# CoderLSF/fast-llama

Measured on AMD Instinct MI355X. Metric: decode tokens/s LLaMA2-7B int8, higher is better.
Workload: dtype int8; 1 GPU; LLaMA2-7B int8 .flm-layout synthetic weights (portable splitmix64 checkpoint, norm weights 1.0), single-stream greedy decode, prompt 9 tokens, positions 14..928, fp32 KV cache, max_seq 1024; parallelism=single-gpu

## Files before the change

fast-llama_amd/capi.py:

```python
from __future__ import annotations

import ctypes as C
import os

import numpy as np

_HERE = os.path.dirname(os.path.abspath(__file__))
LIB_PATH = os.environ.get("FLM_GPU_LIB") or os.path.join(_HERE, "lib", "libflm_gpu.so")

QT_NONE, QT_INT16, QT_INT8 = 0, 1, 2
KCLASSES = ("embed", "qkv", "attn", "attn_o", "ffn13", "ffn2", "cls", "argmax", "allreduce", "attn_wo", "ffn", "qkv_attn_wo", "layer", "back", "layers", "token")

SYMBOLS = (
    "flm_comm_unique_id", "flm_ctx_create", "flm_ctx_destroy", "flm_p2p_export", "flm_p2p_import", "flm_last_error", "flm_upload_tensor",
    "flm_forward", "flm_forward_argmax", "flm_decode_greedy", "flm_decode_timed", "flm_decode_timed_each", "flm_last_tokens", "flm_reset_kv", "flm_prepare", "flm_sync",
    "flm_kernel_times", "flm_kernel_bytes", "flm_set_option", "flm_query", "flm_debug_read",
    "flm_op_quantize", "flm_op_matmul_q", "flm_op_rmsnorm", "flm_op_swiglu", "flm_op_rope", "flm_op_softmax",
    "flm_op_attention", "flm_op_expf", "flm_op_math", "flm_op_square_sum", "flm_op_argmax", "flm_op_handoff_litmus", "flm_plan_shards",
)


TUNING_KEYS = ("wg_per_cu", "use_mfma", "tok_preq", "tok_nstq", "back_nst13", "back_nst13_head", "back_nst2", "back_pre13", "back_pre2", "back_ao2", "inject_wait_failure")


class FlmError(RuntimeError):
    pass


class ModelDesc(C.Structure):
    _fields_ = [(n, C.c_int32) for n in ("dim", "hidden_dim", "n_layers", "n_heads", "n_kv_heads", "vocab_size",
                                          "max_seq_len", "quant_type", "quant_group_size")]


class ShardPlan(C.Structure):
    _fields_ = [(n, C.c_int32) for n in ("head_begin", "head_count", "hidden_begin", "hidden_count", "dim_begin", "dim_count", "vocab_begin", "vocab_count")]


_lib = None


def lib():
    global _lib
    if _lib is None:
        if not os.path.exists(LIB_PATH):
            raise FlmError(f"{LIB_PATH} is missing: run `python -c 'import __graft_entry__ as g; g.build()'` (no CPU fallback exists)")
        _lib = C.CDLL(LIB_PATH, mode=C.RTLD_GLOBAL)
        _lib.flm_last_error.restype = C.c_char_p
        _lib.flm_last_error.argtypes = [C.c_void_p]
    return _lib


def _p(a):
    return a.ctypes.data_as(C.c_void_p) if a is not None else None


def _check(rc, ctx=None):
    if rc != 0:
        msg = lib().flm_last_error(ctx)
        raise FlmError(f"flm error {rc}: {msg.decode() if msg else ''}")


def desc_from_config(cfg, max_seq_len=1024) -> ModelDesc:
    return ModelDesc(cfg.dim, cfg.hidden_dim, cfg.n_layers, cfg.n_heads, cfg.n_kv_heads, cfg.vocab_size,
                     max_seq_len, cfg.quant_type, cfg.quant_group_size)


def plan_shards(desc: ModelDesc, rank: int, world: int) -> ShardPlan:
    out = ShardPlan()
    _check(lib().flm_plan_shards(C.byref(desc), rank, world, C.byref(out)))
    return out


def comm_unique_id() -> bytes:
    buf = C.create_string_buffer(128)
    _check(lib().flm_comm_unique_id(buf))
    return buf.raw


class Ctx:

    def __init__(self, desc: ModelDesc, device=0, rank=0, world=1, comm_id: bytes | None = None):
        self.desc = desc
        self._h = C.c_void_p()
        _check(lib().flm_ctx_create(C.byref(desc), device, rank, world, comm_id, C.byref(self._h)))

    def close(self):
        if self._h:
            lib().flm_ctx_destroy(self._h)
            self._h = C.c_void_p()

    def __del__(self):
        try:
            self.close()
        except Exception:
            pass

    def p2p_export(self) -> bytes:
        buf = C.create_string_buffer(128)
        _check(lib().flm_p2p_export(self._h, buf), self._h)
        return buf.raw

    def p2p_import(self, blobs):
        raw = b"".join(blobs)
        _check(lib().flm_p2p_import(self._h, raw, len(blobs)), self._h)

    @staticmethod
    def regroup(ctxs):
        blobs = [c.p2p_export() for c in ctxs]
        for c in ctxs:
            c.p2p_import(blobs)

    def upload(self, kind, layer, value):
        if isinstance(value, tuple):
            q, s = value
            q = np.ascontiguousarray(q); s = np.ascontiguousarray(s, dtype=np.float32)
            qt = QT_INT8 if q.dtype == np.int8 else QT_INT16
            _check(lib().flm_upload_tensor(self._h, kind, layer, qt, _p(q), _p(s), q.shape[0], q.shape[1]), self._h)
        else:
            v = np.ascontiguousarray(value, dtype=np.float32)
            rows, cols = v.shape if v.ndim == 2 else (1, v.shape[0])
            _check(lib().flm_upload_tensor(self._h, kind, layer, QT_NONE, _p(v), None, rows, cols), self._h)

    def upload_all(self, tensors):
        for (kind, layer), v in tensors.items():
            self.upload(kind, layer, v)

    def forward(self, tokens, pos) -> np.ndarray:
        t = np.ascontiguousarray(tokens, dtype=np.int32)
        out = np.empty(self.desc.vocab_size, dtype=np.float32)
        _check(lib().flm_forward(self._h, _p(t), len(t), int(pos), _p(out)), self._h)
        return out

    def forward_argmax(self, tokens, pos) -> int:
        t = np.ascontiguousarray(tokens, dtype=np.int32)
        nxt = C.c_int32(-1)
        _check(lib().flm_forward_argmax(self._h, _p(t), len(t), int(pos), C.byref(nxt)), self._h)
        return nxt.value

    def decode_greedy(self, first_token, pos, n_steps) -> np.ndarray:
        out = np.empty(n_steps, dtype=np.int32)
        _check(lib().flm_decode_greedy(self._h, int(first_token), int(pos), int(n_steps), _p(out)), self._h)
        return out

    def decode_timed(self, first_token, pos, n_steps) -> float:
        ms = C.c_float(0)
        _check(lib().flm_decode_timed(self._h, int(first_token), int(pos), int(n_steps), C.byref(ms)), self._h)
        return ms.value

    def decode_timed_each(self, first_token, pos, n_steps) -> np.ndarray:
        ms = np.zeros(n_steps, dtype=np.float32)
        _check(lib().flm_decode_timed_each(self._h, int(first_token), int(pos), int(n_steps), _p(ms)), self._h)
        return ms

    def last_tokens(self, n) -> np.ndarray:
        out = np.empty(n, dtype=np.int32)
        _check(lib().flm_last_tokens(self._h, int(n), _p(out)), self._h)
        return out

    def reset_kv(self):
        _check(lib().flm_reset_kv(self._h), self._h)

    def prepare(self):
        _check(lib().flm_prepare(self._h), self._h)

    def sync(self):
        _check(lib().flm_sync(self._h), self._h)

    def set_option(self, key, value, unlock=True):
        if unlock and key in TUNING_KEYS and not self.query("tuning"):
            _check(lib().flm_set_option(self._h, b"tuning", 1), self._h)
        _check(lib().flm_set_option(self._h, key.encode(), int(value)), self._h)

    def query(self, key) -> int:
        v = C.c_int(0)
        _check(lib().flm_query(self._h, key.encode(), C.byref(v)), self._h)
        return int(v.value)

    def debug_read(self, what, layer, n):
        names = {"x1": 0, "q": 1, "att_out": 2, "hd": 3, "kcache": 4, "vcache": 5, "logits": 6, "trace": 7, "trace_abs": 8, "back_trace": 10}
        out = np.empty(n, dtype=np.float32)
        _check(lib().flm_debug_read(self._h, names[what], int(layer), _p(out), C.c_size_t(n)), self._h)
        return out

    def kernel_times(self, pos, iters=3):
        avg = np.zeros(len(KCLASSES), dtype=np.float32); cnt = np.zeros(len(KCLASSES), dtype=np.int32)
        _check(lib().flm_kernel_times(self._h, int(pos), int(iters), _p(avg), _p(cnt)), self._h)
        return {k: (float(avg[i]), int(cnt[i])) for i, k in enumerate(KCLASSES)}

    def kernel_bytes(self, kclass, pos) -> float:
        b = C.c_double(0)
        _check(lib().flm_kernel_bytes(self._h, KCLASSES.index(kclass), int(pos), C.byref(b)), self._h)
        return b.value


def op_quantize(x, qt, gs=64):
    x = np.ascontiguousarray(x, dtype=np.float32)
    q = np.empty(x.size, dtype=np.int8 if qt == QT_INT8 else np.int16)
    s = np.empty(x.size // gs, dtype=np.float32)
    _check(lib().flm_op_quantize(qt, _p(q), _p(s), _p(x), C.c_size_t(x.size), gs))
    return q, s


def op_matmul_q(qt, W, sW, X, sX, gs=64):
    W = np.ascontiguousarray(W); X = np.ascontiguousarray(X)
    sW = np.ascontiguousarray(sW, dtype=np.float32); sX = np.ascontiguousarray(sX, dtype=np.float32)
    m, n = W.shape; w = X.shape[0]
    out = np.empty((w, m), dtype=np.float32)
    _check(lib().flm_op_matmul_q(qt, _p(out), _p(W), _p(sW), _p(X), _p(sX), m, n, w, gs))
    return out


def op_argmax(logits) -> int:
    a = np.ascontiguousarray(logits, dtype=np.float32)
    idx = C.c_int32(-1)
    _check(lib().flm_op_argmax(_p(a), int(a.size), C.byref(idx)))
    return idx.value


def op_handoff_litmus(rounds):
    bad, to = C.c_int(0), C.c_int(0)
    _check(lib().flm_op_handoff_litmus(int(rounds), C.byref(bad), C.byref(to)))
    return bad.value, to.value


def op_rmsnorm(x, w):
    x = np.ascontiguousarray(x, dtype=np.float32); w = np.ascontiguousarray(w, dtype=np.float32)
    o = np.empty_like(x)
    _check(lib().flm_op_rmsnorm(_p(o), _p(x), _p(w), C.c_size_t(x.size)))
    return o


def op_square_sum(x):
    x = np.ascontiguousarray(x, dtype=np.float32)
    o = np.empty(6, dtype=np.float32)
    _check(lib().flm_op_square_sum(_p(x), C.c_size_t(x.size), _p(o)))
    return o[0], o[1], o[2:6]


def op_swiglu(xo, xr):
    a = np.array(xo, dtype=np.float32, copy=True); b = np.ascontiguousarray(xr, dtype=np.float32)
    _check(lib().flm_op_swiglu(_p(a), _p(b), C.c_size_t(a.size)))
    return a


def op_rope(x, pos):
    x = np.ascontiguousarray(x, dtype=np.float32); o = np.empty_like(x)
    _check(lib().flm_op_rope(_p(o), _p(x), x.size, int(pos)))
    return o


def op_softmax(x, n=None):
    a = np.array(x, dtype=np.float32, copy=True)
    _check(lib().flm_op_softmax(_p(a), int(a.size if n is None else n)))
    return a


def op_expf(x):
    a = np.array(x, dtype=np.float32, copy=True).reshape(-1)
    _check(lib().flm_op_expf(_p(a), C.c_size_t(a.size)))
    return a


def op_math(fn, x, y=None):
    a = np.array(x, dtype=np.float32, copy=True).reshape(-1)
    b = None if y is None else np.ascontiguousarray(y, dtype=np.float32).reshape(-1)
    _check(lib().flm_op_math(int(fn), _p(a), _p(b), C.c_size_t(a.size)))
    return a


def op_attention(kc, vc, q, k, v, n_heads, hs, max_seq, pos):
    out = np.empty(n_heads * hs, dtype=np.float32)
    for a in (kc, vc):
        assert a.dtype == np.float32 and a.flags.c_contiguous
    q = np.ascontiguousarray(q, dtype=np.float32); k = np.ascontiguousarray(k, dtype=np.float32); v = np.ascontiguousarray(v, dtype=np.float32)
    _check(lib().flm_op_attention(_p(out), _p(kc), _p(vc), _p(q), _p(k), _p(v), n_heads, hs, max_seq, int(pos)))
    return out
```

fast-llama_amd/csrc/flm_gemv.h:

```cpp
#pragma once
#include "flm_math.h"
#pragma clang fp contract(off)

namespace flm {

struct GemvArgs {
    const void*  W;   const float* sW;
    int n;
    int items;
    int rows_per_pass;
    int cb_shift;
    int ctr_off;
    int nbuf;
    const float* x;
    const float* norm_w;
    const void*  xq; const float* xs;
    float* out;
    float* kcache; float* vcache;
    const float* rope_cos; const float* rope_sin;
    const int* pos_ptr;
    int dim; int kv_dim; int max_seq; int hs;
    float* out_peer[7]; int n_peer;
    unsigned long long* gout; unsigned long long* gout_peer[7];
    unsigned long long* gk; unsigned long long* gv;
// ... 4 lines not shown
    } xf;
    void* dbg_xq; float* dbg_xs; float* dbg_xn;
    unsigned long long* trace;
    int ablate;
};

__device__ __forceinline__ void st_result(const GemvArgs& a, unsigned row, float v) {
    st_agent(a.out + row, v);
    for (int i = 0; i < a.n_peer; ++i) __hip_atomic_store(a.out_peer[i] + row, v, __ATOMIC_RELAXED, __HIP_MEMORY_SCOPE_SYSTEM);
}

#ifndef FLM_ABLATE
#define FLM_ABLATE 0
#endif
constexpr bool kAblate = FLM_ABLATE != 0;
constexpr int kStepBlk = 4;

__host__ __device__ inline int chain_bshift(int n) { int s = 2; while ((64 << s) < n / 4) ++s; return s; }
__host__ __device__ inline int chain_strip_floats(int n) { return 64 * ((1 << chain_bshift(n)) + 4); }
struct GemvLds {
    int off_xs, off_red, off_ctr, off_scr;
    int gstride;
    int buf_bytes;
    int total;
};
__host__ __device__ inline GemvLds gemv_lds_layout(int n, int esz, bool norm, int Rm, int RB, bool two, int nbuf = 2) {
    GemvLds L;
    const int sn = n / kGroup, ng = two ? 2 * sn : sn;
    L.off_xs = n * esz;
    L.off_red = L.off_xs + ((sn * 4 + 15) & ~15);
    L.off_ctr = L.off_red + 64;
    L.off_scr = L.off_ctr + 16;
    int g16 = (ng * 8 + 15) / 16; if ((g16 & 1) == 0) ++g16;
    L.gstride = g16 * 16;
    L.buf_bytes = (Rm + RB) * L.gstride;
    int scratch = nbuf * L.buf_bytes + 64;
    const int chain = 4 * chain_strip_floats(n) * 4 + 64;
    if (norm && chain > scratch) scratch = chain;
    L.total = L.off_scr + scratch;
    return L;
}
__device__ __forceinline__ float sq_chain(const float* p, int n4) {
    float l = 0.f;
    int k = 0;
#define FLM_SQ4(v) l = __fmaf_rn(v.x, v.x, l); l = __fmaf_rn(v.y, v.y, l); l = __fmaf_rn(v.z, v.z, l); l = __fmaf_rn(v.w, v.w, l);
#define FLM_RD4(a, b, c, d, base) a = *reinterpret_cast<const float4*>(pp + (base)); b = *reinterpret_cast<const float4*>(pp + (base) + 4); c = *reinterpret_cast<const float4*>(pp + (base) + 8); d = *reinterpret_cast<const float4*>(pp + (base) + 12);
    if (n4 >= 32) {
        const float* pp = p;
        float4 a0, a1, a2, a3, b0, b1, b2, b3;
        FLM_RD4(a0, a1, a2, a3, 0)
#pragma unroll 2
        for (; k + 32 <= n4; k += 32, pp += 32) {
            FLM_RD4(b0, b1, b2, b3, 16)
            __builtin_amdgcn_s_waitcnt(0xC47F);
            __builtin_amdgcn_sched_barrier(0);
            FLM_SQ4(a0) FLM_SQ4(a1) FLM_SQ4(a2) FLM_SQ4(a3)
            __builtin_amdgcn_sched_barrier(0);
            FLM_RD4(a0, a1, a2, a3, 32)
            __builtin_amdgcn_s_waitcnt(0xC47F);
            __builtin_amdgcn_sched_barrier(0);
            FLM_SQ4(b0) FLM_SQ4(b1) FLM_SQ4(b2) FLM_SQ4(b3)
            __builtin_amdgcn_sched_barrier(0);
        }
        if (k + 4 <= n4) { FLM_SQ4(a0) k += 4; } if (k + 4 <= n4) { FLM_SQ4(a1) k += 4; } if (k + 4 <= n4) { FLM_SQ4(a2) k += 4; } if (k + 4 <= n4) { FLM_SQ4(a3) k += 4; }
    }
#undef FLM_RD4
#undef FLM_SQ4
    for (; k < n4; ++k) l = __fmaf_rn(p[k], p[k], l);
    return l;
}

__device__ __forceinline__ double wave_scan_incl_f64(double v) {
#define FLM_SCAN64(ctrl, rmask, bc) { const int lo_ = __builtin_amdgcn_update_dpp(0, __double2loint(v), ctrl, rmask, 0xF, bc), hi_ = __builtin_amdgcn_update_dpp(0, __double2hiint(v), ctrl, rmask, 0xF, bc); v = __dadd_rn(v, __hiloint2double(hi_, lo_)); }
    FLM_SCAN64(0x111 , 0xF, true) FLM_SCAN64(0x112 , 0xF, true)
    FLM_SCAN64(0x114 , 0xF, true) FLM_SCAN64(0x118 , 0xF, true)
    FLM_SCAN64(0x142 , 0xA, false) FLM_SCAN64(0x143 , 0xC, false)
#undef FLM_SCAN64
    return v;
}
__device__ __forceinline__ float wave_scan_incl(float v) {
#define FLM_SCAN_STEP(ctrl, rmask, bc) v = __fadd_rn(v, __int_as_float(__builtin_amdgcn_update_dpp(0, __float_as_int(v), ctrl, rmask, 0xF, bc)));
    FLM_SCAN_STEP(0x111 , 0xF, true) FLM_SCAN_STEP(0x112 , 0xF, true)
    FLM_SCAN_STEP(0x114 , 0xF, true) FLM_SCAN_STEP(0x118 , 0xF, true)
    FLM_SCAN_STEP(0x142 , 0xA, false) FLM_SCAN_STEP(0x143 , 0xC, false)
#undef FLM_SCAN_STEP
    return v;
}
__device__ __forceinline__ double readlane_f64(double v, int l) {
    return __hiloint2double(__builtin_amdgcn_readlane(__double2hiint(v), l), __builtin_amdgcn_readlane(__double2loint(v), l));
}
constexpr int kChainHead = 4;
#ifdef FLM_TRACE_PRO_RT
#define FLM_CHAIN_STAMP(k) if (tr && lane == 0) tr[k] = __builtin_amdgcn_s_memtime();
#else
#define FLM_CHAIN_STAMP(k)
#endif
template <int OP> __device__ __forceinline__ float chain_step(float l, float x) { if constexpr (OP == 0) return __fmaf_rn(x, x, l); else return __fadd_rn(l, x); }
template <int BVR, int OP = 0, int PAD = 4>
__device__ __forceinline__ float chain_spec_t(const float* p, const int bshift, int* rounds_out, unsigned long long* tr = nullptr, const int Brt = 0) {
    const int lane = threadIdx.x & 63, B = BVR ? 4 * BVR : (Brt ? Brt : (1 << bshift)), BV = B >> 2, LS = B + PAD;
    const float4* pl = reinterpret_cast<const float4*>(p + lane * LS);
    float4 xr[BVR ? BVR : 1];
    if constexpr (BVR > 0) {
#pragma unroll
        for (int q = 0; q < BVR; ++q) xr[q] = pl[q];
    }
    auto elem = [&](int q) -> float4 { if constexpr (BVR > 0) return xr[q]; else return pl[q]; };
    FLM_CHAIN_STAMP(0)
#define FLM_SQ4(l, v) l = chain_step<OP>(l, v.x); l = chain_step<OP>(l, v.y); l = chain_step<OP>(l, v.z); l = chain_step<OP>(l, v.w);
    float s = 0.f; unsigned orb = 0u;
#pragma unroll
    for (int q = 0; q < BV; ++q) { const float4 v = elem(q); FLM_SQ4(s, v) orb |= __float_as_uint(v.x) | __float_as_uint(v.y); orb |= __float_as_uint(v.z) | __float_as_uint(v.w); }
    const bool allzero = (orb & 0x7fffffffu) == 0u;
    const float P = __int_as_float(__builtin_amdgcn_update_dpp(0, __float_as_int(wave_scan_incl(s)), 0x138 , 0xF, 0xF, true));
    FLM_CHAIN_STAMP(1)
    float hv;
    {
        float l = 0.f;
#pragma unroll
        for (int L = 0; L < kChainHead; ++L) {
#pragma unroll
            for (int q = 0; q < BV; ++q) { const float4 v = elem(q); FLM_SQ4(l, v) }
            if (L + 1 < kChainHead) l = __int_as_float(__builtin_amdgcn_update_dpp(0, __float_as_int(l), 0x138 , 0xF, 0xF, true));
        }
        hv = __int_as_float(__builtin_amdgcn_readlane(__float_as_int(l), kChainHead - 1));
    }
    FLM_CHAIN_STAMP(2)
    const unsigned eb = __float_as_uint(P) & 0x7f800000u;
    bool valid = lane >= kChainHead && eb >= (27u << 23) && eb <= (250u << 23);
    const unsigned ebv = valid ? eb : 0x3f800000u;
    const float A = __uint_as_float(ebv), u1 = __uint_as_float(ebv - (23u << 23)), top = __fadd_rn(A, A);
    float ca = A, cb = __fadd_rn(A, u1);
#pragma unroll
    for (int q = 0; q < BV; ++q) { const float4 v = elem(q); FLM_SQ4(ca, v) FLM_SQ4(cb, v) }
    float T = __fsub_rn(ca, A);
    const bool tie = __fsub_rn(cb, ca) != u1;
    if (!(T < INFINITY)) valid = false;
    if (!valid) T = 0.f;
    FLM_CHAIN_STAMP(3)
    const unsigned long long live = __ballot(valid && !allzero);
    bool plain = false;
    if (live) {
        const unsigned e0 = (unsigned)__builtin_amdgcn_readlane((int)eb, __ffsll((long long)live) - 1), e1 = (unsigned)__builtin_amdgcn_readlane((int)eb, 63 - __clzll((long long)live));
        plain = e1 < e0 || ((e1 - e0) >> 23) > 26;
    }
    if (plain) {
        float l = 0.f;
        for (int L = 0; L < 64; ++L) { const float4* r = reinterpret_cast<const float4*>(p + L * LS); for (int q = 0; q < BV; ++q) { const float4 v = r[q]; FLM_SQ4(l, v) } }
        if (rounds_out) *rounds_out = -1;
        return l;
    }
    const double Td = (double)T, Si = wave_scan_incl_f64(Td), S = __dsub_rn(Si, Td);
    FLM_CHAIN_STAMP(4)
    int rounds = 0;
    const unsigned long long zero_m = __ballot(allzero), good_m = __ballot(valid && !tie);
    unsigned long long done_m = (1ull << kChainHead) - 1ull;
    double bv = (double)hv, Sb = readlane_f64(S, kChainHead);
    float res;
    for (;;) {
        ++rounds;
        if (rounds <= 9) { FLM_CHAIN_STAMP(4 + rounds) }
        const float st = (float)__dadd_rn(bv, __dsub_rn(S, Sb));
        const unsigned long long e_m = __ballot((__float_as_uint(st) & 0x7f800000u) == eb), t_m = __ballot(__fadd_rn(st, T) < top);
        const unsigned long long bad = ~(zero_m | (good_m & e_m & t_m) | done_m);
        if (bad == 0) { res = __uint_as_float((unsigned)__builtin_amdgcn_readlane((int)__float_as_uint((float)__dadd_rn(bv, __dsub_rn(Si, Sb))), 63)); break; }
        const int f = __ffsll((long long)bad) - 1;
        float l = st;
#pragma unroll
        for (int q = 0; q < BV; ++q) { const float4 v = elem(q); FLM_SQ4(l, v) }
        res = __uint_as_float((unsigned)__builtin_amdgcn_readlane((int)__float_as_uint(l), f));
        if (f == 63) break;
        done_m = (2ull << f) - 1ull; bv = (double)res; Sb = readlane_f64(S, f + 1);
    }
#undef FLM_SQ4
    FLM_CHAIN_STAMP(14)
    if (tr && lane == 0) tr[15] = (unsigned long long)rounds;
    if (rounds_out) *rounds_out = rounds;
    return res;
}
template <int BVR>
__device__ __forceinline__ float sq_chain_spec_t(const float* p, const int bshift, int* rounds_out, unsigned long long* tr = nullptr) { return chain_spec_t<BVR, 0, 4>(p, bshift, rounds_out, tr); }
__device__ __forceinline__ float sq_chain_spec(const float* p, const int bshift, int* rounds_out = nullptr, unsigned long long* tr = nullptr) {
    return sq_chain_spec_t<0>(p, bshift, rounds_out, tr);
}

template <int QT, int PRO, int XR, bool COH = false>
__device__ __forceinline__ void gemv_preload(const GemvArgs& a, float4 (&xv)[XR > 0 ? XR : 1], float4 (&wv)[XR > 0 ? XR : 1], const float* xsrc = nullptr) {
    if constexpr (PRO == PRO_QUANT || PRO == PRO_RMSNORM_QUANT) {
        typedef float v4f __attribute__((ext_vector_type(4)));
        const __amdgpu_buffer_rsrc_t rx = __builtin_amdgcn_make_buffer_rsrc(const_cast<float*>(xsrc ? xsrc : a.x), 0, a.n * 4, 0x00020000);
        const __amdgpu_buffer_rsrc_t rn = __builtin_amdgcn_make_buffer_rsrc(const_cast<float*>(PRO == PRO_RMSNORM_QUANT ? a.norm_w : a.x), 0, a.n * 4, 0x00020000);
#pragma unroll
        for (int i = 0; i < XR; ++i) {
            const int off = (threadIdx.x * 4 + i * kGemvBlock * 4) * 4;
            const v4f v = __builtin_bit_cast(v4f, __builtin_amdgcn_raw_buffer_load_b128(rx, off, 0, COH ? kAuxCoherent : 0));
            xv[i] = make_float4(v.x, v.y, v.z, v.w);
            if constexpr (PRO == PRO_RMSNORM_QUANT) {
                const v4f u = __builtin_bit_cast(v4f, __builtin_amdgcn_raw_buffer_load_b128(rn, off, 0, 0));
                wv[i] = make_float4(u.x, u.y, u.z, u.w);
            }
        }
    }
}

typedef unsigned v4u_g __attribute__((ext_vector_type(4)));
typedef unsigned long long granule_t;
__device__ __forceinline__ void st_granule(granule_t* g, unsigned tag, float v) {
    __hip_atomic_store(g, ((granule_t)tag << 32) | (granule_t)__float_as_uint(v), __ATOMIC_RELAXED, __HIP_MEMORY_SCOPE_AGENT);
}
__device__ __forceinline__ float ld_granule_value(const granule_t* g) { return __uint_as_float((unsigned)__hip_atomic_load(g, __ATOMIC_RELAXED, __HIP_MEMORY_SCOPE_AGENT)); }
__device__ __forceinline__ void st_result_granule(const GemvArgs& a, unsigned row, unsigned tag, float v) {
    st_granule(a.gout + row, tag, v);
    const granule_t g = ((granule_t)tag << 32) | (granule_t)__float_as_uint(v);
    for (int i = 0; i < a.n_peer; ++i) __hip_atomic_store(a.gout_peer[i] + row, g, __ATOMIC_RELAXED, __HIP_MEMORY_SCOPE_SYSTEM);
}

#ifndef FLM_QUANT_SHARED_RCP
#define FLM_QUANT_SHARED_RCP 1
#endif
template <int QT>
__device__ __forceinline__ void quant_round4(char* xq, float* xs, int e, bool act, const float4& v) {
    using T = QTraits<QT>;
    const float mx = row16_max(fmaxf(fmaxf(fabsf(v.x), fabsf(v.y)), fmaxf(fabsf(v.z), fabsf(v.w))));
    const float sc = __fdiv_rn(mx, T::kF);
    int qq[4];
#if FLM_QUANT_SHARED_RCP
    quant_elems4(v, sc, qq);
#else
    qq[0] = quant_elem(v.x, sc); qq[1] = quant_elem(v.y, sc); qq[2] = quant_elem(v.z, sc); qq[3] = quant_elem(v.w, sc);
#endif
    if (act) {
        const int q0 = qq[0], q1 = qq[1], q2 = qq[2], q3 = qq[3];
        if constexpr (QT == QT_INT8) {
            const uint32_t pk = (uint32_t)(q0 & 0xff) | ((uint32_t)(q1 & 0xff) << 8) | ((uint32_t)(q2 & 0xff) << 16) | ((uint32_t)(q3 & 0xff) << 24);
            *reinterpret_cast<uint32_t*>(xq + e) = pk;
        } else {
            uint2 pk;
            pk.x = (uint32_t)(q0 & 0xffff) | ((uint32_t)(q1 & 0xffff) << 16);
            pk.y = (uint32_t)(q2 & 0xffff) | ((uint32_t)(q3 & 0xffff) << 16);
            *reinterpret_cast<uint2*>(xq + (size_t)e * 2) = pk;
        }
        if ((threadIdx.x & 15) == 0) xs[e / kGroup] = sc;
    }
}

#ifdef FLM_TRACE_PRO_RT
#define FLM_PRO_STAMP(k) if (kAblate && a.trace && (threadIdx.x == 0 || threadIdx.x == 960)) a.trace[blockIdx.x * 16 + (threadIdx.x ? 8 : 0) + (k)] = __builtin_amdgcn_s_memrealtime();
#elif defined(FLM_TRACE_PRO)
#define FLM_PRO_STAMP(k) if (kAblate && a.trace && threadIdx.x == 0) a.trace[blockIdx.x * 8 + (k)] = __builtin_amdgcn_s_memtime();
#else
#define FLM_PRO_STAMP(k)
#endif
template <int QT, int PRO, int XR, bool COH = false, bool LATE = false, class AfterStage>
__device__ __forceinline__ void gemv_prologue(const GemvArgs& a, char* lds, float4 (&xv)[XR > 0 ? XR : 1], float4 (&wv)[XR > 0 ? XR : 1], AfterStage&& after_stage) {
    using T = QTraits<QT>;
    const int n = a.n;
    const int tid = threadIdx.x;
    const GemvLds L = gemv_lds_layout(n, T::kEsz, PRO == PRO_RMSNORM_QUANT, a.rows_per_pass, 64 >> a.cb_shift, false);
    char*  xq = lds;
    float* xs = reinterpret_cast<float*>(lds + L.off_xs);
    float* red = reinterpret_cast<float*>(lds + L.off_red);
    float* scratch = reinterpret_cast<float*>(lds + L.off_scr);

    if constexpr (PRO == PRO_NONE) {
        const int nb16 = n * T::kEsz / 16;
        if constexpr (COH) {
            const __amdgpu_buffer_rsrc_t rq = __builtin_amdgcn_make_buffer_rsrc(const_cast<void*>(a.xq), 0, n * T::kEsz, 0x00020000);
            for (int c = tid; c < nb16; c += kGemvBlock)
                reinterpret_cast<v4i*>(xq)[c] = __builtin_bit_cast(v4i, __builtin_amdgcn_raw_buffer_load_b128(rq, c * 16, 0, kAuxCoherent));
            for (int g = tid; g < n / kGroup; g += kGemvBlock) xs[g] = ld_agent(a.xs + g);
        } else {
            for (int c = tid; c < nb16; c += kGemvBlock)
                reinterpret_cast<int4*>(xq)[c] = reinterpret_cast<const int4*>(a.xq)[c];
            for (int g = tid; g < n / kGroup; g += kGemvBlock) xs[g] = a.xs[g];
        }
        __syncthreads();
        return;
    } else {
        const int rounds = (n + kGemvBlock * 4 - 1) / (kGemvBlock * 4);
        const float4 z4 = make_float4(0.f, 0.f, 0.f, 0.f);
        float r = 1.0f;
#ifdef FLM_TRACE_PRO_RT
        FLM_PRO_STAMP(0)
#endif
        auto ldx = [&](int e) -> float4 {
            if constexpr (COH) {
                typedef float v4f __attribute__((ext_vector_type(4)));
                const __amdgpu_buffer_rsrc_t rx = __builtin_amdgcn_make_buffer_rsrc(const_cast<float*>(a.x), 0, n * 4, 0x00020000);
                const v4f t = __builtin_bit_cast(v4f, __builtin_amdgcn_raw_buffer_load_b128(rx, e * 4, 0, kAuxCoherent));
                return make_float4(t.x, t.y, t.z, t.w);
            } else return *reinterpret_cast<const float4*>(a.x + e);
        };
        if constexpr (PRO == PRO_QUANT) {
            if constexpr (XR > 0) { asm volatile("" :: "v"(xv[XR - 1].w)); }
            FLM_PRO_STAMP(3)
            if constexpr (!LATE) after_stage(0);
            FLM_PRO_STAMP(4)
        }
        if constexpr (PRO == PRO_RMSNORM_QUANT) {
            const int bs = chain_bshift(n), B = 1 << bs, LS = B + 4, CS = 64 * LS, slots = 64 << bs;
            auto stage = [&](int i, const float4& v) {
                const int k = tid + i * kGemvBlock;
                if (k < slots) { const int o = (k >> bs) * LS + (k & (B - 1)); scratch[o] = v.x; scratch[CS + o] = v.y; scratch[2 * CS + o] = v.z; scratch[3 * CS + o] = v.w; }
            };
            const int srounds = (slots + kGemvBlock - 1) / kGemvBlock;
#pragma unroll
            for (int i = 0; i < XR; ++i) { if (i < srounds) stage(i, xv[i]); }
            for (int i = XR; i < srounds; ++i) {
                const int e = tid * 4 + i * kGemvBlock * 4;
                stage(i, e < n ? ldx(e) : z4);
            }
#ifdef FLM_TRACE_PRO_RT
            FLM_PRO_STAMP(1)
#endif
            __syncthreads();
            FLM_PRO_STAMP(3)
            if constexpr (!LATE) {
                if (tid >= 4 * kWave) __builtin_amdgcn_s_sleep(2);
                after_stage(0);
#ifdef FLM_TRACE_PRO2
                FLM_PRO_STAMP(1)
#endif
                if (tid < 4 * kWave && !(kAblate && (a.ablate & 2))) {
                    const float l = sq_chain_spec(scratch + (tid >> 6) * CS, bs);
                    if ((tid & 63) == 0) red[8 + (tid >> 6)] = l;
// ... 538 lines not shown
```

fast-llama_amd/csrc/flm_ops.hip:

```cpp
#include "flm_host.h"

namespace {
struct DevBuf {
    void* p = nullptr;
    ~DevBuf() { if (p) hipFree(p); }
    int alloc(size_t n) { return hipMalloc(&p, n ? n : 4) == hipSuccess ? 0 : 1; }
    template <class T> T* as() { return reinterpret_cast<T*>(p); }
};
#define OPC(expr) do { hipError_t e_ = (expr); if (e_ != hipSuccess) { g_last_error = std::string(#expr " failed: ") + hipGetErrorString(e_); return FLM_ERR_HIP; } } while (0)
}

extern "C" {


int flm_op_quantize(int qt, void* qx, float* qs, const float* x, size_t n, int gs) {
    if (!qx || !qs || !x || gs != kGroup || n % kGroup) return FLM_ERR_INVALID;
    if (qt != FLM_QT_INT8 && qt != FLM_QT_INT16) return FLM_ERR_UNSUPPORTED;
    const int e = esz_of(qt);
    DevBuf dx, dq, ds;
    if (dx.alloc(n * 4) || dq.alloc(n * e) || ds.alloc(n / kGroup * 4)) return FLM_ERR_OOM;
    OPC(hipMemcpy(dx.p, x, n * 4, hipMemcpyHostToDevice));
    if (n <= 16384) {
        GemvArgs a{}; a.n = (int)n; a.items = 0; a.x = dx.as<float>(); a.dbg_xq = dq.p; a.dbg_xs = ds.as<float>();
        int r = launch_gemv<PRO_QUANT, EPI_STORE>(nullptr, 0, qt, a, 1); if (r) return r;
    } else {
        int r = quantize_flat(nullptr, 0, qt, dq.p, ds.as<float>(), dx.as<float>(), n); if (r) return r;
    }
    OPC(hipDeviceSynchronize());
    OPC(hipMemcpy(qx, dq.p, n * e, hipMemcpyDeviceToHost));
    OPC(hipMemcpy(qs, ds.p, n / kGroup * 4, hipMemcpyDeviceToHost));
    return FLM_OK;
}

int flm_op_square_sum(const float* x, size_t n, float* out6) {
    if (!x || !out6 || n % 16 || n == 0 || n > 16384) return FLM_ERR_INVALID;
    DevBuf dx, dout;
    if (dx.alloc(n * 4) || dout.alloc(16 * 4)) return FLM_ERR_OOM;
    OPC(hipMemcpy(dx.p, x, n * 4, hipMemcpyHostToDevice));
    const size_t lds = ((size_t)4 * chain_strip_floats((int)n) + 4 * (n / 4 + 8)) * 4;
    hipLaunchKernelGGL(k_op_square_sum, dim3(1), dim3(256), lds, 0, dout.as<float>(), dx.as<float>(), (int)n);
    OPC(hipGetLastError()); OPC(hipDeviceSynchronize());
    OPC(hipMemcpy(out6, dout.p, 6 * 4, hipMemcpyDeviceToHost));
    if (getenv("FLM_SQ_ITERS")) { float it[6]; hipMemcpy(it, (char*)dout.p + 24, 24, hipMemcpyDeviceToHost); fprintf(stderr, "sq_chain_spec rounds per chain (-1: plain chain): %g %g %g %g; shader-clock ticks: speculative %g, plain %g\n", it[0], it[1], it[2], it[3], it[4], it[5]); }
    return FLM_OK;
}

int flm_op_handoff_litmus(int rounds, int* wrong_values, int* timed_out) {
    if (rounds < 1 || !wrong_values || !timed_out) return FLM_ERR_INVALID;
    int dev = 0; OPC(hipGetDevice(&dev));
    hipDeviceProp_t pr; OPC(hipGetDeviceProperties(&pr, dev));
    const int G = pr.multiProcessorCount < 256 ? pr.multiProcessorCount : 256;
    DevBuf pay, fl, er;
    if (pay.alloc((size_t)2 * G * 64 * 4) || fl.alloc((size_t)G * 64) || er.alloc(8)) return FLM_ERR_OOM;
    OPC(hipMemset(pay.p, 0, (size_t)2 * G * 64 * 4)); OPC(hipMemset(fl.p, 0, (size_t)G * 64)); OPC(hipMemset(er.p, 0, 8));
    hipLaunchKernelGGL(k_handoff_litmus, dim3(G), dim3(256), 0, 0, pay.as<float>(), fl.as<unsigned>(), rounds, er.as<int>(), er.as<int>() + 1);
    OPC(hipGetLastError()); OPC(hipDeviceSynchronize());
    int h[2] = {0, 0};
    OPC(hipMemcpy(h, er.p, 8, hipMemcpyDeviceToHost));
    *wrong_values = h[0]; *timed_out = h[1];
    return FLM_OK;
}

int flm_op_rmsnorm(float* o, const float* x, const float* w, size_t n) {
    if (!o || !x || !w || n % kGroup || n > 16384 || n == 0) return FLM_ERR_INVALID;
    DevBuf dx, dw, dn, dq, ds;
    if (dx.alloc(n * 4) || dw.alloc(n * 4) || dn.alloc(n * 4) || dq.alloc(n) || ds.alloc(n / kGroup * 4)) return FLM_ERR_OOM;
    OPC(hipMemcpy(dx.p, x, n * 4, hipMemcpyHostToDevice)); OPC(hipMemcpy(dw.p, w, n * 4, hipMemcpyHostToDevice));
    GemvArgs a{}; a.n = (int)n; a.items = 0; a.x = dx.as<float>(); a.norm_w = dw.as<float>();
    a.dbg_xn = dn.as<float>(); a.dbg_xq = dq.p; a.dbg_xs = ds.as<float>();
    int r = launch_gemv<PRO_RMSNORM_QUANT, EPI_STORE>(nullptr, 0, FLM_QT_INT8, a, 1); if (r) return r;
    OPC(hipDeviceSynchronize());
    OPC(hipMemcpy(o, dn.p, n * 4, hipMemcpyDeviceToHost));
    return FLM_OK;
}

int flm_op_matmul_q(int qt, float* out, const void* W, const float* sW, const void* X, const float* sX, int m, int n, int w, int gs) {
    if (!out || !W || !sW || !X || !sX || m < 1 || n < 1 || w < 1 || gs != kGroup || n % kGroup) return FLM_ERR_INVALID;
    if (qt != FLM_QT_INT8 && qt != FLM_QT_INT16) return FLM_ERR_UNSUPPORTED;
    const size_t e = esz_of(qt), sn = n / kGroup;
    DevBuf dW, dsW, dX, dsX, dsXT, dsWT, dO;
    if (dW.alloc((size_t)m * n * e) || dsW.alloc((size_t)m * sn * 4) || dX.alloc((size_t)w * n * e) || dsX.alloc((size_t)w * sn * 4) || dsXT.alloc((size_t)w * sn * 4 + 64) || dsWT.alloc((size_t)m * sn * 4) || dO.alloc((size_t)w * m * 4)) return FLM_ERR_OOM;
    {
        std::vector<float> t((size_t)w * sn);
        for (int b = 0; b < w; ++b) for (size_t g = 0; g < sn; ++g) t[g * w + b] = sX[(size_t)b * sn + g];
        OPC(hipMemcpy(dsXT.p, t.data(), t.size() * 4, hipMemcpyHostToDevice));
        std::vector<float> tw((size_t)m * sn);
        for (int r = 0; r < m; ++r) for (size_t g = 0; g < sn; ++g) tw[g * m + r] = sW[(size_t)r * sn + g];
        OPC(hipMemcpy(dsWT.p, tw.data(), tw.size() * 4, hipMemcpyHostToDevice));
    }
    OPC(hipMemcpy(dW.p, W, (size_t)m * n * e, hipMemcpyHostToDevice)); OPC(hipMemcpy(dsW.p, sW, (size_t)m * sn * 4, hipMemcpyHostToDevice));
    OPC(hipMemcpy(dX.p, X, (size_t)w * n * e, hipMemcpyHostToDevice)); OPC(hipMemcpy(dsX.p, sX, (size_t)w * sn * 4, hipMemcpyHostToDevice));
    int dev = 0, cus = 256; hipGetDevice(&dev); hipDeviceGetAttribute(&cus, hipDeviceAttributeMultiprocessorCount, dev);
    const char* gv = getenv("FLM_OP_GEMM");
    if (w >= 16 && !(gv && !strcmp(gv, "gemv"))) {
        GemmArgs g{dW.p, dsW.as<float>(), dX.p, dsX.as<float>(), dO.as<float>(), m, n, m, w, dsXT.as<float>(), dsWT.as<float>()};
        const int um = gv ? atoi(gv) : 1;
        int r = launch_gemm_store(nullptr, 0, qt, g, um);
        if (r) return r;
    } else {
        for (int b = 0; b < w; ++b) {
            GemvArgs a{}; a.W = dW.p; a.sW = dsW.as<float>(); a.n = n; a.items = m;
            a.xq = (const char*)dX.p + (size_t)b * n * e; a.xs = dsX.as<float>() + (size_t)b * sn; a.out = dO.as<float>() + (size_t)b * m;
            int r = launch_gemv<PRO_NONE, EPI_STORE>(nullptr, 0, qt, a, gemv_grid(cus, 1, m, 1)); if (r) return r;
        }
    }
    OPC(hipDeviceSynchronize());
    OPC(hipMemcpy(out, dO.p, (size_t)w * m * 4, hipMemcpyDeviceToHost));
    return FLM_OK;
}

int flm_op_argmax(const float* logits, int n, int32_t* idx) {
    if (!logits || !idx || n < 1) return FLM_ERR_INVALID;
    DevBuf dl, dst, dout;
    if (dl.alloc((size_t)n * 4) || dst.alloc(sizeof(DecodeState)) || dout.alloc(16)) return FLM_ERR_OOM;
    OPC(hipMemcpy(dl.p, logits, (size_t)n * 4, hipMemcpyHostToDevice));
    OPC(hipMemset(dst.p, 0, sizeof(DecodeState)));
    hipLaunchKernelGGL(k_argmax_advance, dim3(1), dim3(1024), 0, 0, (const float*)dl.as<float>(), n, dst.as<DecodeState>(), dout.as<int>(), 0, 4);
    OPC(hipGetLastError()); OPC(hipDeviceSynchronize());
    OPC(hipMemcpy(idx, dout.p, 4, hipMemcpyDeviceToHost));
    return FLM_OK;
}

int flm_op_swiglu(float* xo, const float* xr, size_t n) {
    if (!xo || !xr || n == 0) return FLM_ERR_INVALID;
    DevBuf a, b; if (a.alloc(n * 4) || b.alloc(n * 4)) return FLM_ERR_OOM;
    OPC(hipMemcpy(a.p, xo, n * 4, hipMemcpyHostToDevice)); OPC(hipMemcpy(b.p, xr, n * 4, hipMemcpyHostToDevice));
    hipLaunchKernelGGL(k_op_swiglu, dim3(256), dim3(256), 0, 0, a.as<float>(), (const float*)b.as<float>(), n);
    OPC(hipGetLastError()); OPC(hipDeviceSynchronize());
    OPC(hipMemcpy(xo, a.p, n * 4, hipMemcpyDeviceToHost));
    return FLM_OK;
}

int flm_op_rope(float* o, const float* x, int n_dims, int pos) {
    if (!o || !x || n_dims < 2 || n_dims % 2 || pos < 0) return FLM_ERR_INVALID;
    std::vector<float> cs, sn; build_rope_table(n_dims, pos + 1, cs, sn);
    DevBuf dx, dout, dc, dsn; const size_t h = n_dims / 2;
    if (dx.alloc(n_dims * 4) || dout.alloc(n_dims * 4) || dc.alloc(h * 4) || dsn.alloc(h * 4)) return FLM_ERR_OOM;
    OPC(hipMemcpy(dx.p, x, n_dims * 4, hipMemcpyHostToDevice));
    OPC(hipMemcpy(dc.p, cs.data() + (size_t)pos * h, h * 4, hipMemcpyHostToDevice)); OPC(hipMemcpy(dsn.p, sn.data() + (size_t)pos * h, h * 4, hipMemcpyHostToDevice));
    hipLaunchKernelGGL(k_op_rope, dim3((unsigned)((h + 63) / 64)), dim3(64), 0, 0, dout.as<float>(), (const float*)dx.as<float>(), n_dims, (const float*)dc.as<float>(), (const float*)dsn.as<float>());
    OPC(hipGetLastError()); OPC(hipDeviceSynchronize());
    OPC(hipMemcpy(o, dout.p, n_dims * 4, hipMemcpyDeviceToHost));
    return FLM_OK;
}

int flm_op_softmax(float* x, int n) {
    if (!x || n < 1) return FLM_ERR_INVALID;
    DevBuf d; if (d.alloc((size_t)n * 4)) return FLM_ERR_OOM;
    OPC(hipMemcpy(d.p, x, (size_t)n * 4, hipMemcpyHostToDevice));
    hipLaunchKernelGGL(k_op_softmax, dim3(1), dim3(kBlock), 0, 0, d.as<float>(), n);
    OPC(hipGetLastError()); OPC(hipDeviceSynchronize());
    OPC(hipMemcpy(x, d.p, (size_t)n * 4, hipMemcpyDeviceToHost));
    return FLM_OK;
}

int flm_op_attention(float* out, float* kc, float* vc, const float* q, const float* k, const float* v,
                     int n_heads, int hs, int max_seq, int pos) {
    if (!out || !kc || !vc || !q || !k || !v || n_heads < 1 || hs < 32 || hs > 256 || hs % 8 || pos < 0 || pos >= max_seq) return FLM_ERR_INVALID;
    const size_t nd = (size_t)n_heads * hs, nc = (size_t)n_heads * max_seq * hs, h2 = hs / 2;
    std::vector<float> cs, sn; build_rope_table(hs, pos + 1, cs, sn);
    DevBuf dq, dk, dv, dkc, dvc, dout, dc, dsn, dpos;
    if (dq.alloc(nd * 4) || dk.alloc(nd * 4) || dv.alloc(nd * 4) || dkc.alloc(nc * 4) || dvc.alloc(nc * 4) || dout.alloc(nd * 4) ||
        dc.alloc(h2 * 4) || dsn.alloc(h2 * 4) || dpos.alloc(4)) return FLM_ERR_OOM;
    OPC(hipMemcpy(dq.p, q, nd * 4, hipMemcpyHostToDevice)); OPC(hipMemcpy(dk.p, k, nd * 4, hipMemcpyHostToDevice)); OPC(hipMemcpy(dv.p, v, nd * 4, hipMemcpyHostToDevice));
    OPC(hipMemcpy(dkc.p, kc, nc * 4, hipMemcpyHostToDevice)); OPC(hipMemcpy(dvc.p, vc, nc * 4, hipMemcpyHostToDevice));
    OPC(hipMemcpy(dc.p, cs.data() + (size_t)pos * h2, h2 * 4, hipMemcpyHostToDevice)); OPC(hipMemcpy(dsn.p, sn.data() + (size_t)pos * h2, h2 * 4, hipMemcpyHostToDevice));
    OPC(hipMemcpy(dpos.p, &pos, 4, hipMemcpyHostToDevice));
    hipLaunchKernelGGL(k_op_kv_append, dim3((unsigned)((nd / 2 + 255) / 256)), dim3(256), 0, 0, dq.as<float>(), (const float*)dk.as<float>(), (const float*)dv.as<float>(),
                       dkc.as<float>(), dvc.as<float>(), (const float*)dc.as<float>(), (const float*)dsn.as<float>(), n_heads, hs, max_seq, pos);
    OPC(hipGetLastError());
    AttnArgs a{}; a.q = dq.as<float>(); a.kcache = dkc.as<float>(); a.vcache = dvc.as<float>(); a.pos_ptr = dpos.as<int>(); a.hs = hs; a.max_seq = max_seq;
    a.out = dout.as<float>();
    int G = (getenv("FLM_OP_ATTN_PARTS") && atoi(getenv("FLM_OP_ATTN_PARTS")) > 1) ? hs / kSplitDims : 1;
    if (G < 2 || hs % kSplitDims || hs > 128 || n_heads * G > 256 || max_seq > kSplitMaxSeq) G = 1;
    DevBuf dsc, dfl, derr;
    if (dsc.alloc((size_t)n_heads * max_seq * 4) || dfl.alloc(256 * 64) || derr.alloc(64)) return FLM_ERR_OOM;
    OPC(hipMemset(dfl.p, 0, 256 * 64)); OPC(hipMemset(derr.p, 0, 64));
    a.G = G; a.sc_global = dsc.as<float>(); a.flag_sc = dfl.as<unsigned>(); a.epoch = 1; a.err = derr.as<int>();
    if (G > 1) hipLaunchKernelGGL(k_attn_decode<true>, dim3(n_heads * G), dim3(kAttnBlock), attn_lds_bytes(max_seq, hs, true), 0, a);
    else       hipLaunchKernelGGL(k_attn_decode<false>, dim3(n_heads), dim3(kAttnBlock), attn_lds_bytes(max_seq, hs, false), 0, a);
    OPC(hipGetLastError());
    OPC(hipDeviceSynchronize());
    OPC(hipMemcpy(out, dout.p, nd * 4, hipMemcpyDeviceToHost));
    OPC(hipMemcpy(kc, dkc.p, nc * 4, hipMemcpyDeviceToHost)); OPC(hipMemcpy(vc, dvc.p, nc * 4, hipMemcpyDeviceToHost));
    return FLM_OK;
}

int flm_op_math(int fn, float* x, const float* y, size_t n) {
    if (!x || n == 0 || fn < 0 || fn > 5 || (fn >= 2 && !y)) return FLM_ERR_INVALID;
    DevBuf d, e; if (d.alloc(n * 4) || e.alloc(n * 4)) return FLM_ERR_OOM;
    OPC(hipMemcpy(d.p, x, n * 4, hipMemcpyHostToDevice));
    if (y) OPC(hipMemcpy(e.p, y, n * 4, hipMemcpyHostToDevice));
    hipLaunchKernelGGL(k_op_math, dim3(1024), dim3(256), 0, 0, fn, d.as<float>(), (const float*)e.as<float>(), n);
    OPC(hipGetLastError()); OPC(hipDeviceSynchronize());
    OPC(hipMemcpy(x, d.p, n * 4, hipMemcpyDeviceToHost));
    return FLM_OK;
// ... 5 lines not shown
```

include/flm_gpu.h:

```cpp
#ifndef FLM_GPU_H
#define FLM_GPU_H
#include <stddef.h>
#include <stdint.h>
#ifdef __cplusplus
extern "C" {
#endif

#define FLM_OK               0
#define FLM_ERR_INVALID     -1
#define FLM_ERR_UNSUPPORTED -2
#define FLM_ERR_HIP         -3
#define FLM_ERR_OOM         -4
#define FLM_ERR_STATE       -5
#define FLM_ERR_COMM        -6

#define FLM_QT_NONE  0
#define FLM_QT_INT16 1
#define FLM_QT_INT8  2

#define FLM_T_TOKEN_EMBD  1
#define FLM_T_OUTPUT_NORM 2
#define FLM_T_CLASSIFIER  3
#define FLM_T_INPUT_NORM 17
#define FLM_T_ATTN_Q     18
#define FLM_T_ATTN_K     19
#define FLM_T_ATTN_V     20
#define FLM_T_ATTN_O     21
#define FLM_T_MLP_GATE   22
#define FLM_T_MLP_UP     23
#define FLM_T_MLP_DOWN   24
#define FLM_T_POST_NORM  25

typedef struct flm_ctx flm_ctx;

typedef struct flm_model_desc {
    int32_t dim;
    int32_t hidden_dim;
    int32_t n_layers;
    int32_t n_heads;
    int32_t n_kv_heads;
    int32_t vocab_size;
    int32_t max_seq_len;
    int32_t quant_type;
    int32_t quant_group_size;
} flm_model_desc;

int  flm_comm_unique_id(void* out128);
int  flm_ctx_create(const flm_model_desc* desc, int device_id, int rank, int world,
                    const void* comm_id, flm_ctx** out);
void flm_ctx_destroy(flm_ctx* ctx);
#define FLM_P2P_BLOB_BYTES 128
int  flm_p2p_export(flm_ctx* ctx, void* blob128);
int  flm_p2p_import(flm_ctx* ctx, const void* blobs , int world);
const char* flm_last_error(const flm_ctx* ctx);

int  flm_upload_tensor(flm_ctx* ctx, int kind, int layer, int src_qtype,
                       const void* values, const float* scales, int rows, int cols);
int  flm_prepare(flm_ctx* ctx);

int  flm_forward(flm_ctx* ctx, const int32_t* tokens, int n, int pos, float* logits_host);
int  flm_forward_argmax(flm_ctx* ctx, const int32_t* tokens, int n, int pos, int32_t* next_token);
int  flm_decode_greedy(flm_ctx* ctx, int32_t first_token, int pos, int n_steps, int32_t* out_tokens);
int  flm_decode_timed(flm_ctx* ctx, int32_t first_token, int pos, int n_steps, float* ms);
int  flm_decode_timed_each(flm_ctx* ctx, int32_t first_token, int pos, int n_steps, float* ms_each);
int  flm_last_tokens(flm_ctx* ctx, int n, int32_t* out);
int  flm_reset_kv(flm_ctx* ctx);
int  flm_sync(flm_ctx* ctx);

#define FLM_KCLASSES 16
int  flm_kernel_times(flm_ctx* ctx, int pos, int iters, float* avg_us, int32_t* count);
int  flm_kernel_bytes(flm_ctx* ctx, int kclass, int pos, double* bytes);

int  flm_debug_read(flm_ctx* ctx, int what, int layer, float* out, size_t n);

int  flm_set_option(flm_ctx* ctx, const char* key, int value);
int  flm_query(flm_ctx* ctx, const char* key, int* value);

int  flm_op_quantize(int qt, void* qx, float* qs, const float* x, size_t n, int gs);
int  flm_op_matmul_q(int qt, float* out, const void* mat1, const float* scales1,
                     const void* mat2, const float* scales2, int m, int n, int w, int gs);
int  flm_op_rmsnorm(float* o, const float* x, const float* w, size_t n);
int  flm_op_square_sum(const float* x, size_t n, float* out6);
int  flm_op_argmax(const float* logits, int n, int32_t* idx);
int  flm_op_swiglu(float* xo, const float* xr, size_t n);
int  flm_op_rope(float* o, const float* x, int n_dims, int pos);
int  flm_op_softmax(float* x, int n);
int  flm_op_attention(float* out, float* kc, float* vc, const float* q, const float* k, const float* v,
                      int n_heads, int hs, int max_seq, int pos);
int  flm_op_expf(float* x, size_t n);
int  flm_op_math(int fn, float* x, const float* y, size_t n);
int  flm_op_handoff_litmus(int rounds, int* wrong_values, int* timed_out);

typedef struct flm_shard_plan {
    int32_t head_begin, head_count;
    int32_t hidden_begin, hidden_count;
    int32_t dim_begin, dim_count;
    int32_t vocab_begin, vocab_count;
} flm_shard_plan;
int  flm_plan_shards(const flm_model_desc* desc, int rank, int world, flm_shard_plan* out);

#ifdef __cplusplus
}
#endif
#endif
```

Measured before the change: 557.2 tokens/s.

## Walk predicted-bad lanes before verification pass in speculative square-sum chain

Result: no change. 556.9 tokens/s, median of 2 (-0.0%).

```diff
diff --git a/fast-llama_amd/capi.py b/fast-llama_amd/capi.py
--- a/fast-llama_amd/capi.py
+++ b/fast-llama_amd/capi.py
@@ -16,7 +16,7 @@
     "flm_forward", "flm_forward_argmax", "flm_decode_greedy", "flm_decode_timed", "flm_decode_timed_each", "flm_last_tokens", "flm_reset_kv", "flm_prepare", "flm_sync",
     "flm_kernel_times", "flm_kernel_bytes", "flm_set_option", "flm_query", "flm_debug_read",
     "flm_op_quantize", "flm_op_matmul_q", "flm_op_rmsnorm", "flm_op_swiglu", "flm_op_rope", "flm_op_softmax",
-    "flm_op_attention", "flm_op_expf", "flm_op_math", "flm_op_square_sum", "flm_op_argmax", "flm_op_handoff_litmus", "flm_plan_shards",
+    "flm_op_attention", "flm_op_expf", "flm_op_math", "flm_op_square_sum", "flm_op_square_sum_rounds", "flm_op_argmax", "flm_op_handoff_litmus", "flm_plan_shards",
 )
 
 
@@ -237,6 +237,13 @@
     return o[0], o[1], o[2:6]
 
 
+def op_square_sum_rounds(x):
+    x = np.ascontiguousarray(x, dtype=np.float32)
+    o = np.empty(6, dtype=np.float32); r = np.empty(4, dtype=np.int32)
+    _check(lib().flm_op_square_sum_rounds(_p(x), C.c_size_t(x.size), _p(o), _p(r)))
+    return o[0], o[1], o[2:6], r
+
+
 def op_swiglu(xo, xr):
     a = np.array(xo, dtype=np.float32, copy=True); b = np.ascontiguousarray(xr, dtype=np.float32)
     _check(lib().flm_op_swiglu(_p(a), _p(b), C.c_size_t(a.size)))
diff --git a/fast-llama_amd/csrc/flm_gemv.h b/fast-llama_amd/csrc/flm_gemv.h
--- a/fast-llama_amd/csrc/flm_gemv.h
+++ b/fast-llama_amd/csrc/flm_gemv.h
@@ -180,25 +180,48 @@
     }
     const double Td = (double)T, Si = wave_scan_incl_f64(Td), S = __dsub_rn(Si, Td);
     FLM_CHAIN_STAMP(4)
-    int rounds = 0;
+    int rounds = 1;
+    FLM_CHAIN_STAMP(5)
     const unsigned long long zero_m = __ballot(allzero), good_m = __ballot(valid && !tie);
-    unsigned long long done_m = (1ull << kChainHead) - 1ull;
+    const unsigned long long walk_m = __ballot(lane >= kChainHead && !allzero && !(valid && !tie && __fadd_rn(P, s) < top));
     double bv = (double)hv, Sb = readlane_f64(S, kChainHead);
-    float res;
-    for (;;) {
-        ++rounds;
-        if (rounds <= 9) { FLM_CHAIN_STAMP(4 + rounds) }
+    float res = hv, stv = 0.f;
+    int last = kChainHead - 1;
+    for (unsigned long long w = walk_m; w; w &= w - 1ull) {
+        const int c = __ffsll((long long)w) - 1;
+        float l = (float)__dadd_rn(bv, __dsub_rn(S, Sb));
+        stv = lane > last ? l : stv;
+#pragma unroll
+        for (int q = 0; q < BV; ++q) { const float4 v = elem(q); FLM_SQ4(l, v) }
+        res = __uint_as_float((unsigned)__builtin_amdgcn_readlane((int)__float_as_uint(l), c));
+        last = c; bv = (double)res; Sb = readlane_f64(Si, c);
+    }
+    if (last < 63) {
         const float st = (float)__dadd_rn(bv, __dsub_rn(S, Sb));
-        const unsigned long long e_m = __ballot((__float_as_uint(st) & 0x7f800000u) == eb), t_m = __ballot(__fadd_rn(st, T) < top);
-        const unsigned long long bad = ~(zero_m | (good_m & e_m & t_m) | done_m);
-        if (bad == 0) { res = __uint_as_float((unsigned)__builtin_amdgcn_readlane((int)__float_as_uint((float)__dadd_rn(bv, __dsub_rn(Si, Sb))), 63)); break; }
-        const int f = __ffsll((long long)bad) - 1;
-        float l = st;
-#pragma unroll
-        for (int q = 0; q < BV; ++q) { const float4 v = elem(q); FLM_SQ4(l, v) }
-        res = __uint_as_float((unsigned)__builtin_amdgcn_readlane((int)__float_as_uint(l), f));
-        if (f == 63) break;
-        done_m = (2ull << f) - 1ull; bv = (double)res; Sb = readlane_f64(S, f + 1);
+        stv = lane > last ? st : stv;
+        res = __uint_as_float((unsigned)__builtin_amdgcn_readlane((int)__float_as_uint((float)__dadd_rn(bv, __dsub_rn(Si, Sb))), 63));
+    }
+    const unsigned long long pass_bad = ~(zero_m | walk_m | ((1ull << kChainHead) - 1ull) |
+                                          (good_m & __ballot((__float_as_uint(stv) & 0x7f800000u) == eb) & __ballot(__fadd_rn(stv, T) < top)));
+    if (pass_bad) {
+        const int f0 = __ffsll((long long)pass_bad) - 1;
+        unsigned long long done_m = (1ull << f0) - 1ull;
+        bv = (double)__uint_as_float((unsigned)__builtin_amdgcn_readlane((int)__float_as_uint(stv), f0)); Sb = readlane_f64(S, f0);
+        for (;;) {
+            ++rounds;
+            if (rounds <= 9) { FLM_CHAIN_STAMP(4 + rounds) }
+            const float st = (float)__dadd_rn(bv, __dsub_rn(S, Sb));
+            const unsigned long long e_m = __ballot((__float_as_uint(st) & 0x7f800000u) == eb), t_m = __ballot(__fadd_rn(st, T) < top);
+            const unsigned long long bad = ~(zero_m | (good_m & e_m & t_m) | done_m);
+            if (bad == 0) { res = __uint_as_float((unsigned)__builtin_amdgcn_readlane((int)__float_as_uint((float)__dadd_rn(bv, __dsub_rn(Si, Sb))), 63)); break; }
+            const int f = __ffsll((long long)bad) - 1;
+            float l = st;
+#pragma unroll
+            for (int q = 0; q < BV; ++q) { const float4 v = elem(q); FLM_SQ4(l, v) }
+            res = __uint_as_float((unsigned)__builtin_amdgcn_readlane((int)__float_as_uint(l), f));
+            if (f == 63) break;
+            done_m = (2ull << f) - 1ull; bv = (double)res; Sb = readlane_f64(S, f + 1);
+        }
     }
 #undef FLM_SQ4
     FLM_CHAIN_STAMP(14)
diff --git a/fast-llama_amd/csrc/flm_ops.hip b/fast-llama_amd/csrc/flm_ops.hip
--- a/fast-llama_amd/csrc/flm_ops.hip
+++ b/fast-llama_amd/csrc/flm_ops.hip
@@ -42,6 +42,20 @@
     OPC(hipGetLastError()); OPC(hipDeviceSynchronize());
     OPC(hipMemcpy(out6, dout.p, 6 * 4, hipMemcpyDeviceToHost));
     if (getenv("FLM_SQ_ITERS")) { float it[6]; hipMemcpy(it, (char*)dout.p + 24, 24, hipMemcpyDeviceToHost); fprintf(stderr, "sq_chain_spec rounds per chain (-1: plain chain): %g %g %g %g; shader-clock ticks: speculative %g, plain %g\n", it[0], it[1], it[2], it[3], it[4], it[5]); }
+    return FLM_OK;
+}
+int flm_op_square_sum_rounds(const float* x, size_t n, float* out6, int* rounds4) {
+    if (!x || !out6 || !rounds4 || n % 16 || n == 0 || n > 16384) return FLM_ERR_INVALID;
+    DevBuf dx, dout;
+    if (dx.alloc(n * 4) || dout.alloc(16 * 4)) return FLM_ERR_OOM;
+    OPC(hipMemcpy(dx.p, x, n * 4, hipMemcpyHostToDevice));
+    const size_t lds = ((size_t)4 * chain_strip_floats((int)n) + 4 * (n / 4 + 8)) * 4;
+    hipLaunchKernelGGL(k_op_square_sum, dim3(1), dim3(256), lds, 0, dout.as<float>(), dx.as<float>(), (int)n);
+    OPC(hipGetLastError()); OPC(hipDeviceSynchronize());
+    float o[10];
+    OPC(hipMemcpy(o, dout.p, 10 * 4, hipMemcpyDeviceToHost));
+    for (int i = 0; i < 6; ++i) out6[i] = o[i];
+    for (int i = 0; i < 4; ++i) rounds4[i] = (int)o[6 + i];
     return FLM_OK;
 }
 
diff --git a/include/flm_gpu.h b/include/flm_gpu.h
--- a/include/flm_gpu.h
+++ b/include/flm_gpu.h
@@ -81,6 +81,7 @@
                      const void* mat2, const float* scales2, int m, int n, int w, int gs);
 int  flm_op_rmsnorm(float* o, const float* x, const float* w, size_t n);
 int  flm_op_square_sum(const float* x, size_t n, float* out6);
+int  flm_op_square_sum_rounds(const float* x, size_t n, float* out6, int* rounds4);
 int  flm_op_argmax(const float* logits, int n, int32_t* idx);
 int  flm_op_swiglu(float* xo, const float* xr, size_t n);
 int  flm_op_rope(float* o, const float* x, int n_dims, int pos);
```
